# Wangkkklll/GausPcc

Hardware: AMD Instinct MI355X
Metric: Mpoints/s encode+decode @1M anchors (higher is better)
Workload: dtype f32

## Files before the change

gauspcc_amd/csrc/rangecoder_dev.hpp:

```cpp
#pragma once
#include "rangecoder.hpp"

namespace gpcc {

__device__ __forceinline__ int clz32(uint32_t x) { return x ? __clz((int)x) : 32; }

constexpr int RING_NPH = 3;

__device__ __forceinline__ uint32_t scale(uint64_t span, uint32_t v) { return (uint32_t)((span * (uint64_t)v) >> 16); }
__device__ __forceinline__ uint32_t scale_d(uint32_t d, uint32_t v)
{
#ifdef RC_SCALE_MUL64
    return (uint32_t)(((uint64_t)d * (uint64_t)v + (uint64_t)v) >> 16);
#else
    const uint32_t dh = d >> 16, dl = d & 0xFFFFu;
    return __umul24(dh, v) + ((__umul24(dl, v) + v) >> 16);
#endif
}

__device__ __forceinline__ uint32_t ones_below(uint32_t k) { return (1u << (k & 31u)) - 1u; }

struct LaneWin {
    const uint32_t *w;
    uint32_t q;
    uint32_t w0, w1;
    uint32_t last;
    __device__ __forceinline__ void init(const uint32_t *p, uint32_t rdw) { w = p; q = 31u; w0 = p[0]; w1 = p[1]; last = rdw - 2u; }
    __device__ __forceinline__ uint32_t peek() const { return __builtin_amdgcn_alignbit(w0, w1, ~q); }
    __device__ __forceinline__ void advance(uint32_t k) { q += k; const uint32_t i = min(q >> 5, last); w0 = w[i]; w1 = w[i + 1u]; }
};

__device__ __forceinline__ void stage_windows(uint32_t *win, const uint8_t *__restrict__ bytes, const RcChunk &ch, int nl, uint32_t rdw, int nthreads, int owner_stride, int lane)
{
    const uint32_t total = (uint32_t)nl * rdw;
    const uint32_t nbf = ch.nbytes;
    for (uint32_t f0 = 0; f0 < total; f0 += 4u * (uint32_t)nthreads) {
        uint32_t v[4];
#pragma unroll
        for (int u = 0; u < 4; ++u) {
            const uint32_t f = f0 + (uint32_t)u * (uint32_t)nthreads + (uint32_t)lane;
            const uint32_t j = min(f / rdw, (uint32_t)nl - 1u), dq = f - (f / rdw) * rdw;
            const uint32_t off = (uint32_t)__shfl((int)ch.byte_off, (int)j * owner_stride, 64);
            const uint32_t nb = (uint32_t)__shfl((int)nbf, (int)j * owner_stride, 64);
            const bool back = (nb & RC_BACKWARDS) != 0u;
            const uint32_t n = nb & ~RC_BACKWARDS;
            uint32_t raw = 0;
            if (f < total && 4u * dq < n) {
                const uint8_t *src = back ? bytes + (size_t)off - 4u * (size_t)dq - 3u : bytes + (size_t)off + 4u * (size_t)dq;
                __builtin_memcpy(&raw, src, 4);
                if (!back) raw = __builtin_bswap32(raw);
                const uint32_t left = n - 4u * dq;
                if (left < 4u) raw &= 0xFFFFFFFFu << (8u * (4u - left));
            }
            v[u] = raw;
        }
#pragma unroll
        for (int u = 0; u < 4; ++u) {
            const uint32_t f = f0 + (uint32_t)u * (uint32_t)nthreads + (uint32_t)lane;
            if (f < total) win[f] = v[u];
        }
    }
}

__device__ __forceinline__ uint32_t ffbh(uint32_t v) { uint32_t r; asm("v_ffbh_u32_e32 %0, %1" : "=v"(r) : "v"(v)); return r; }
__device__ __forceinline__ void rc_renorm(uint32_t &low, uint32_t &d, uint32_t &x, uint32_t lo, uint32_t d1, uint32_t t, uint32_t &k_out)
{
    const uint32_t x1 = x - lo, low1 = low + lo, high1 = low1 + d1;
    const uint32_t n1 = ffbh(low1 ^ high1);
    const uint32_t l1 = low1 << n1, h1 = (high1 << n1) | ~(0xFFFFFFFFu << n1);
    const uint32_t n2 = ffbh((((~l1) | h1) << 1) | 1u);
    const uint32_t k = n1 + n2;
    low = (l1 << n2) & 0x7FFFFFFFu;
    d = (d1 << k) | ~(0xFFFFFFFFu << k);
    x = (uint32_t)(((((uint64_t)x1) << 32 | (uint64_t)t) << k) >> 32);
    k_out = k;
}

__device__ __forceinline__ void cp_renorm(uint32_t &range, uint32_t &x, uint32_t lo, uint32_t r1, uint32_t t, uint32_t &k_out)
{
    const uint32_t x1 = x - lo;
    const uint32_t k = ffbh(r1 | 0x8000u);
    range = r1 << k;
    x = (uint32_t)(((((uint64_t)x1) << 32 | (uint64_t)t) << k) >> 32);
    k_out = k;
}

constexpr int RC_CODER_CARRYLESS = 0, RC_CODER_CARRY = 1;
__host__ __device__ inline int rc_coder_of_version(int version) { return version >= 4 ? RC_CODER_CARRY : RC_CODER_CARRYLESS; }

template <bool SOLO> __device__ __forceinline__ void rc_wave_sync()
{
    if (SOLO) __syncthreads();
    else { asm volatile("s_waitcnt lgkmcnt(0)" ::: "memory"); __builtin_amdgcn_wave_barrier(); }
}

template <int LP, int PH, bool SOLO, int CODER = RC_CODER_CARRYLESS>
__device__ __forceinline__ void rc_decode_lds_wave(const uint16_t *cdf, const uint8_t *__restrict__ bytes, const RcChunk *__restrict__ chunks,
                                                   int nchunks, int c0, int lane, int lpw, uint32_t rdw, uint8_t *sym, uint32_t *win)
{
    static_assert(LP == 3 || LP == 5, "17-entry rows are decoded by rc_decode17_lds_wave");
    static_assert(PH == 16 || PH == 4, "phase length");
    constexpr int RS = LP == 3 ? 1 : 4;
    constexpr int DEPTH = RING_NPH * PH;
    const int c = c0 + lane;
    RcChunk ch = {0, 0, 0, 0, 0, 0};
    if (lane < lpw && c < nchunks) ch = chunks[c];
    uint32_t nmax = ch.n;
#pragma unroll
    for (int d = 32; d >= 1; d >>= 1) nmax = max(nmax, (uint32_t)__shfl_xor((int)nmax, d));
    nmax = (uint32_t)__builtin_amdgcn_readfirstlane((int)nmax);
    if (nmax == 0) return;
    stage_windows(win, bytes, ch, lpw, rdw, 64, 1, lane);
    rc_wave_sync<SOLO>();
    LaneWin in;
    in.init(win + (size_t)min(lane, lpw - 1) * rdw, rdw);
    const uint16_t *rowp = cdf + (size_t)ch.first * RS;
    const size_t rstep = (size_t)ch.stride * RS;
    struct Row { uint32_t a, b; };
    Row regs[RING_NPH][PH];
    auto fill = [&](int h) {
#pragma unroll
        for (int dd = 0; dd < PH; ++dd) {
            if (LP == 3) { regs[h][dd].a = rowp[0]; regs[h][dd].b = 0; }
            else { const uint2 q = *reinterpret_cast<const uint2 *>(rowp); regs[h][dd].a = q.x; regs[h][dd].b = q.y; }
            rowp += rstep;
        }
    };
    uint32_t low = 0, d = 0xFFFFFFFFu, x = in.w0, k;
#pragma unroll
    for (int h = 0; h < RING_NPH; ++h) fill(h);
    uint8_t *out = sym + ch.out;
    for (uint32_t i0 = 0; i0 < nmax; i0 += DEPTH) {
#pragma unroll
        for (int h = 0; h < RING_NPH; ++h) {
            uint32_t pack[PH / 4];
#pragma unroll
            for (int dd = 0; dd < PH; ++dd) {
                const uint32_t r0 = regs[h][dd].a, r1 = regs[h][dd].b;
                const uint32_t t = in.peek();
                uint32_t s, lo, d1;
                if constexpr (CODER == RC_CODER_CARRY) {
                    const uint32_t r = d >> 16;
                    if (LP == 3) {
                        const uint32_t t1 = __umul24(r, r0);
                        const bool ge = t1 <= x;
                        s = ge; lo = ge ? t1 : 0u;
                        d1 = ge ? d - t1 : t1;
                    } else {
                        const uint32_t t1 = __umul24(r, r0 & 0xFFFFu), t2 = __umul24(r, r0 >> 16), t3 = __umul24(r, r1 & 0xFFFFu);
                        const bool g1 = t1 <= x, g2 = t2 <= x, g3 = t3 <= x;
                        lo = g3 ? t3 : (g2 ? t2 : (g1 ? t1 : 0u));
                        const uint32_t hi = g3 ? d : (g2 ? t3 : (g1 ? t2 : t1));
                        s = (g1 ? 1u : 0u) + (g2 ? 1u : 0u) + (g3 ? 1u : 0u);
                        d1 = hi - lo;
                    }
                    if ((dd & 3) == 0) pack[dd >> 2] = s; else pack[dd >> 2] |= s << (8 * (dd & 3));
                    cp_renorm(d, x, lo, d1, t, k);
                } else {
                if (LP == 3) {
                    const uint32_t t1 = scale_d(d, r0);
                    const bool ge = t1 <= x;
                    s = ge; lo = ge ? t1 : 0u;
                    d1 = ge ? d - t1 : t1 - 1u;
                } else {
                    const uint32_t t1 = scale_d(d, r0 & 0xFFFFu), t2 = scale_d(d, r0 >> 16), t3 = scale_d(d, r1 & 0xFFFFu);
                    const bool g1 = t1 <= x, g2 = t2 <= x, g3 = t3 <= x;
                    lo = g3 ? t3 : (g2 ? t2 : (g1 ? t1 : 0u));
                    const uint32_t hi = g3 ? d + 1u : (g2 ? t3 : (g1 ? t2 : t1));
                    s = (g1 ? 1u : 0u) + (g2 ? 1u : 0u) + (g3 ? 1u : 0u);
                    d1 = hi + ~lo;
                }
                if ((dd & 3) == 0) pack[dd >> 2] = s; else pack[dd >> 2] |= s << (8 * (dd & 3));
                rc_renorm(low, d, x, lo, d1, t, k);
                }
                in.advance(k);
            }
            __builtin_amdgcn_sched_barrier(0);
            if (i0 + (uint32_t)(DEPTH + h * PH) < nmax) fill(h);
            __builtin_amdgcn_sched_barrier(0);
            const uint32_t ib = i0 + (uint32_t)(h * PH);
            bool wide = false;
            if constexpr (PH == 16) {
                wide = ib + 16u <= ch.n;
                if (wide) *reinterpret_cast<uint4 *>(out + ib) = make_uint4(pack[0], pack[1], pack[2], pack[3]);
            }
            if (!wide) {
#pragma unroll
                for (int q = 0; q < PH / 4; ++q)
                    if (ib + 4u * (uint32_t)q < ch.n) *reinterpret_cast<uint32_t *>(out + ib + 4 * q) = pack[q];
            }
        }
    }
}

template <int PH, bool SOLO, int CODER = RC_CODER_CARRYLESS>
__device__ __forceinline__ void rc_decode17_lds_wave(const uint16_t *cdf, const uint8_t *__restrict__ bytes, const RcChunk *__restrict__ chunks,
                                                     int nchunks, int c0, int lane, uint32_t rdw, uint8_t *sym, uint32_t *win)
{
    static_assert(PH == 16 || PH == 4, "phase length");
    constexpr int DEPTH = RING_NPH * PH;
    static_assert(2 * DEPTH <= RC_ROW_LOOKAHEAD, "row look-ahead exceeds the capacity contract (rc_rows_capacity)");
    const int grp = lane >> 4, kk = lane & 15;
    const int c = c0 + grp;
    RcChunk ch = {0, 0, 0, 0, 0, 0};
    if (c < nchunks) ch = chunks[c];
    uint32_t nmax = ch.n;
#pragma unroll
    for (int d = 32; d >= 1; d >>= 1) nmax = max(nmax, (uint32_t)__shfl_xor((int)nmax, d));
    nmax = (uint32_t)__builtin_amdgcn_readfirstlane((int)nmax);
    if (nmax == 0) return;
    stage_windows(win, bytes, ch, 4, rdw, 64, 16, lane);
    rc_wave_sync<SOLO>();
    LaneWin in;
    in.init(win + (size_t)grp * rdw, rdw);
    const uint16_t *rowp = cdf + (size_t)ch.first * 16 + (size_t)(kk ? kk - 1 : 15);
    const size_t rstep = (size_t)ch.stride * 16;
    uint32_t regs[RING_NPH][PH];
    auto fill = [&](int h) {
#pragma unroll
        for (int dd = 0; dd < PH; ++dd) { regs[h][dd] = rowp[0]; rowp += rstep; }
    };
    const int g16 = grp << 4;
    uint32_t low = 0, d = 0xFFFFFFFFu, x = in.w0, k;
#pragma unroll
    for (int h = 0; h < RING_NPH; ++h) fill(h);
    uint8_t *out = sym + ch.out;
    for (uint32_t i0 = 0; i0 < nmax; i0 += DEPTH) {
#pragma unroll
        for (int h = 0; h < RING_NPH; ++h) {
            uint32_t pack[PH / 4];
#pragma unroll
            for (int dd = 0; dd < PH; ++dd) {
                const uint32_t v = regs[h][dd];
                const uint32_t tw = in.peek();
                const uint32_t t = kk ? (CODER == RC_CODER_CARRY ? __umul24(d >> 16, v) : scale_d(d, v)) : 0u;
                const uint64_t bal = __ballot(t <= x);
                const uint32_t half = (grp & 2) ? (uint32_t)(bal >> 32) : (uint32_t)bal;
                const uint32_t bits = (half >> ((grp & 1) * 16)) & 0xFFFFu;
                const uint32_t s = ((uint32_t)__popc(bits) - 1u) & 15u;
                const uint32_t lo = (uint32_t)__shfl((int)t, g16 + (int)s);
                const uint32_t nx = (uint32_t)__shfl((int)t, g16 + (int)min(s + 1u, 15u));
                if ((dd & 3) == 0) pack[dd >> 2] = s; else pack[dd >> 2] |= s << (8 * (dd & 3));
                if constexpr (CODER == RC_CODER_CARRY) {
                    cp_renorm(d, x, lo, (s == 15u ? d : nx) - lo, tw, k);
                } else {
                    const uint32_t d1 = (s == 15u ? d : nx - 1u) - lo;
                    rc_renorm(low, d, x, lo, d1, tw, k);
                }
                in.advance(k);
            }
            __builtin_amdgcn_sched_barrier(0);
            if (i0 + (uint32_t)(DEPTH + h * PH) < nmax) fill(h);
            __builtin_amdgcn_sched_barrier(0);
            const uint32_t ib = i0 + (uint32_t)(h * PH);
            if (kk == 0) {
                bool wide = false;
                if constexpr (PH == 16) {
                    wide = ib + 16u <= ch.n;
                    if (wide) *reinterpret_cast<uint4 *>(out + ib) = make_uint4(pack[0], pack[1], pack[2], pack[3]);
                }
                if (!wide) {
#pragma unroll
                    for (int q = 0; q < PH / 4; ++q)
                        if (ib + 4u * (uint32_t)q < ch.n) *reinterpret_cast<uint32_t *>(out + ib + 4 * q) = pack[q];
                }
            }
        }
    }
}


}
```

Before: 21.18.

## Replace ds_bpermute shuffles with DPP row reductions in 16-lane range decoder

In the 16-lane cooperative decoder, the symbol's low and high bounds now come from DPP row-rotate max and min reductions over the 16-lane row. This replaces two cross-lane shuffles that had to wait on the ballot and popcount result. Lanes are remapped so every lane holds a real CDF threshold, and the popcount uses a 15-bit mask. The narrow-alphabet carry decoder is also rewritten to use subtract-with-overflow and clz, dropping the guard OR, and the bitstream peek is moved next to its use. This shortens the serial dependency chain per symbol but adds eight DPP ops and relies on unguarded clz being nonzero-safe.

```diff
diff --git a/gauspcc_amd/csrc/rangecoder_dev.hpp b/gauspcc_amd/csrc/rangecoder_dev.hpp
--- a/gauspcc_amd/csrc/rangecoder_dev.hpp
+++ b/gauspcc_amd/csrc/rangecoder_dev.hpp
@@ -19,6 +19,16 @@
 }
 
 __device__ __forceinline__ uint32_t ones_below(uint32_t k) { return (1u << (k & 31u)) - 1u; }
+
+template <int N> __device__ __forceinline__ uint32_t row_ror(uint32_t v) { return (uint32_t)__builtin_amdgcn_update_dpp(0, (int)v, 0x120 + N, 0xF, 0xF, false); }
+__device__ __forceinline__ uint32_t row16_max(uint32_t v)
+{
+    v = max(v, row_ror<1>(v)); v = max(v, row_ror<2>(v)); v = max(v, row_ror<4>(v)); return max(v, row_ror<8>(v));
+}
+__device__ __forceinline__ uint32_t row16_min(uint32_t v)
+{
+    v = min(v, row_ror<1>(v)); v = min(v, row_ror<2>(v)); v = min(v, row_ror<4>(v)); return min(v, row_ror<8>(v));
+}
 
 struct LaneWin {
     const uint32_t *w;
@@ -76,10 +86,11 @@
     k_out = k;
 }
 
+template <bool GUARD = true>
 __device__ __forceinline__ void cp_renorm(uint32_t &range, uint32_t &x, uint32_t lo, uint32_t r1, uint32_t t, uint32_t &k_out)
 {
     const uint32_t x1 = x - lo;
-    const uint32_t k = ffbh(r1 | 0x8000u);
+    const uint32_t k = GUARD ? ffbh(r1 | 0x8000u) : (uint32_t)__builtin_clz(r1);
     range = r1 << k;
     x = (uint32_t)(((((uint64_t)x1) << 32 | (uint64_t)t) << k) >> 32);
     k_out = k;
@@ -137,15 +148,18 @@
 #pragma unroll
             for (int dd = 0; dd < PH; ++dd) {
                 const uint32_t r0 = regs[h][dd].a, r1 = regs[h][dd].b;
-                const uint32_t t = in.peek();
                 uint32_t s, lo, d1;
                 if constexpr (CODER == RC_CODER_CARRY) {
                     const uint32_t r = d >> 16;
+                    uint32_t x1;
                     if (LP == 3) {
                         const uint32_t t1 = __umul24(r, r0);
-                        const bool ge = t1 <= x;
-                        s = ge; lo = ge ? t1 : 0u;
-                        d1 = ge ? d - t1 : t1;
+                        uint32_t xm;
+                        const bool lt = __builtin_sub_overflow(x, t1, &xm);
+                        s = lt ? 0u : 1u;
+                        x1 = lt ? x : xm;
+                        d1 = lt ? t1 : d - t1;
+                        k = (uint32_t)__builtin_clz(d1);
                     } else {
                         const uint32_t t1 = __umul24(r, r0 & 0xFFFFu), t2 = __umul24(r, r0 >> 16), t3 = __umul24(r, r1 & 0xFFFFu);
                         const bool g1 = t1 <= x, g2 = t2 <= x, g3 = t3 <= x;
@@ -153,9 +167,12 @@
                         const uint32_t hi = g3 ? d : (g2 ? t3 : (g1 ? t2 : t1));
                         s = (g1 ? 1u : 0u) + (g2 ? 1u : 0u) + (g3 ? 1u : 0u);
                         d1 = hi - lo;
+                        x1 = x - lo;
+                        k = ffbh(d1 | 0x8000u);
                     }
                     if ((dd & 3) == 0) pack[dd >> 2] = s; else pack[dd >> 2] |= s << (8 * (dd & 3));
-                    cp_renorm(d, x, lo, d1, t, k);
+                    d = d1 << k;
+                    x = (uint32_t)(((((uint64_t)x1) << 32 | (uint64_t)in.peek()) << k) >> 32);
                 } else {
                 if (LP == 3) {
                     const uint32_t t1 = scale_d(d, r0);
@@ -171,7 +188,7 @@
                     d1 = hi + ~lo;
                 }
                 if ((dd & 3) == 0) pack[dd >> 2] = s; else pack[dd >> 2] |= s << (8 * (dd & 3));
-                rc_renorm(low, d, x, lo, d1, t, k);
+                rc_renorm(low, d, x, lo, d1, in.peek(), k);
                 }
                 in.advance(k);
             }
@@ -213,14 +230,13 @@
     rc_wave_sync<SOLO>();
     LaneWin in;
     in.init(win + (size_t)grp * rdw, rdw);
-    const uint16_t *rowp = cdf + (size_t)ch.first * 16 + (size_t)(kk ? kk - 1 : 15);
+    const uint16_t *rowp = cdf + (size_t)ch.first * 16 + (size_t)min(kk, 14);
     const size_t rstep = (size_t)ch.stride * 16;
     uint32_t regs[RING_NPH][PH];
     auto fill = [&](int h) {
 #pragma unroll
         for (int dd = 0; dd < PH; ++dd) { regs[h][dd] = rowp[0]; rowp += rstep; }
     };
-    const int g16 = grp << 4;
     uint32_t low = 0, d = 0xFFFFFFFFu, x = in.w0, k;
 #pragma unroll
     for (int h = 0; h < RING_NPH; ++h) fill(h);
@@ -233,20 +249,16 @@
             for (int dd = 0; dd < PH; ++dd) {
                 const uint32_t v = regs[h][dd];
                 const uint32_t tw = in.peek();
-                const uint32_t t = kk ? (CODER == RC_CODER_CARRY ? __umul24(d >> 16, v) : scale_d(d, v)) : 0u;
-                const uint64_t bal = __ballot(t <= x);
+                const uint32_t t = CODER == RC_CODER_CARRY ? __umul24(d >> 16, v) : scale_d(d, v);
+                const bool le = t <= x;
+                const uint32_t lo = row16_max(le ? t : 0u);
+                const uint32_t hi = row16_min(le ? d : (CODER == RC_CODER_CARRY ? t : t - 1u));
+                const uint64_t bal = __ballot(le);
                 const uint32_t half = (grp & 2) ? (uint32_t)(bal >> 32) : (uint32_t)bal;
-                const uint32_t bits = (half >> ((grp & 1) * 16)) & 0xFFFFu;
-                const uint32_t s = ((uint32_t)__popc(bits) - 1u) & 15u;
-                const uint32_t lo = (uint32_t)__shfl((int)t, g16 + (int)s);
-                const uint32_t nx = (uint32_t)__shfl((int)t, g16 + (int)min(s + 1u, 15u));
+                const uint32_t s = (uint32_t)__popc((half >> ((grp & 1) * 16)) & 0x7FFFu);
                 if ((dd & 3) == 0) pack[dd >> 2] = s; else pack[dd >> 2] |= s << (8 * (dd & 3));
-                if constexpr (CODER == RC_CODER_CARRY) {
-                    cp_renorm(d, x, lo, (s == 15u ? d : nx) - lo, tw, k);
-                } else {
-                    const uint32_t d1 = (s == 15u ? d : nx - 1u) - lo;
-                    rc_renorm(low, d, x, lo, d1, tw, k);
-                }
+                if constexpr (CODER == RC_CODER_CARRY) cp_renorm<false>(d, x, lo, hi - lo, tw, k);
+                else rc_renorm(low, d, x, lo, hi - lo, tw, k);
                 in.advance(k);
             }
             __builtin_amdgcn_sched_barrier(0);
```

Result: no change. 21.27 (median of 6 runs) (+0.4%).
